# mic-rud/Learned-Compression-of-Point-Cloud-Geometry-and-Attributes

Hardware: AMD Instinct MI355X
Metric: encode+decode Mpoints/sec (higher is better)
Workload: dtype f32

## Files before the change

### include/pcc_hip.h

```cpp
#ifndef PCC_HIP_H
#define PCC_HIP_H

#include <stdint.h>

#ifdef __cplusplus
extern "C" {
#endif

#define PCC_OK 0
#define PCC_ERR_ARG (-1)
#define PCC_ERR_HIP (-2)
#define PCC_ERR_UNSUPPORTED (-3)
#define PCC_ERR_DATA (-4)

#define PCC_ACT_NONE 0
#define PCC_ACT_RELU 1
#define PCC_ACT_LEAKY_RELU 2

int pcc_version(void);
const char* pcc_last_error(void);
int pcc_device_count(void);
int pcc_device_name(int dev, char* out, int out_len);

int64_t pcc_hash_capacity(int64_t n);

#define PCC_COORD_LIMIT 130000
#define PCC_BATCH_LIMIT 1022
#define PCC_COUNT_ERR_RANGE (-2)

int pcc_hash_build(const int32_t* coords, int64_t n, uint64_t* keys, int32_t* vals, int64_t cap,
                   int32_t tensor_stride, int32_t* dup_count, void* stream);

int pcc_hash_lookup(const uint64_t* keys, const int32_t* vals, int64_t cap, int32_t tensor_stride,
                    const int32_t* query, int64_t nq, int32_t* out_idx, void* stream);

int64_t pcc_scan_scratch_elems(int64_t m);

int pcc_stride_map(const int32_t* coords, int64_t n, int32_t ts, uint64_t* keys, int32_t* vals,
                   int64_t cap, int32_t* scratch, int32_t* out_coords, int64_t* out_count,
                   void* stream);

int pcc_children(const int32_t* coords, int64_t n, int32_t ts, int32_t ksize, uint64_t* keys,
                 int32_t* vals, int64_t cap, int32_t* scratch, int32_t* out_coords,
                 int64_t* out_count, void* stream);

int pcc_kernel_map(const int32_t* out_coords, int64_t n_out, const uint64_t* in_keys,
                   const int32_t* in_vals, int64_t in_cap, int32_t ksize, int32_t step,
                   int32_t sign, int32_t* nbr, uint32_t* row_mask, int64_t* pair_count,
                   void* stream);

int pcc_pair_count(const uint32_t* row_mask, int64_t n_out, int64_t* pair_count, void* stream);

int64_t pcc_order_scratch_bytes(int64_t n);
int pcc_order_rows_by_mask(const uint32_t* row_mask, const int32_t* coords, int64_t n,
                           int32_t block_log2, int32_t tensor_stride, int32_t* order, uint32_t* group_mask32,
                           void* scratch, int64_t scratch_bytes, void* stream);
int pcc_permute_map_rows(const int32_t* nbr, const int32_t* order, int64_t n, int32_t K, int32_t* nbr_sorted, void* stream);

int64_t pcc_small_map_max(void);
int32_t pcc_small_paths(int32_t mask);
int pcc_small_kernel_map(const int32_t* out_coords, int64_t n_out, const uint64_t* in_keys, const int32_t* in_vals, int64_t in_cap,
                         int32_t ksize, int32_t step, int32_t sign, int32_t* nbr, uint32_t* row_mask, int32_t* order,
                         uint32_t* group_mask32, void* scratch, int64_t scratch_bytes, void* stream);

int64_t pcc_conv_packed_elems(int32_t K, int32_t cin, int32_t cout);
int pcc_conv_pack_weights(const float* w, int32_t K, int32_t cin, int32_t cout, float* w_packed,
                          void* stream);
int pcc_conv_fwd(const float* fin, int64_t n_in, int32_t cin, const float* w, const float* w_packed,
                 const float* bias, const int32_t* nbr, const int32_t* order,
                 const uint32_t* group_mask32, int32_t K, float* fout, int64_t n_out, int32_t cout,
                 int32_t act, const float* film, const float* residual, void* stream);

int64_t pcc_conv_small_max(int64_t workgroups);

int pcc_conv_kernel_name(int32_t mode, int64_t n_in, int32_t cin, int32_t cout, int64_t n_out, int32_t K, int32_t has_nbr,
                         char* buf, int32_t len);

int64_t pcc_conv_packed_elems_bf16(int32_t K, int32_t cin, int32_t cout);
int pcc_conv_pack_weights_bf16(const float* w, int32_t K, int32_t cin, int32_t cout, uint16_t* w_packed, void* stream);
int pcc_conv_fwd_bf16(const uint16_t* fin, int64_t n_in, int32_t cin, const uint16_t* w_packed, const float* bias,
                      const int32_t* nbr, const int32_t* order, const uint32_t* group_mask32, int32_t K, float* fout,
                      int64_t n_out, int32_t cout, int32_t act, const float* film, const float* residual, void* stream);

int pcc_epilogue_fwd(const float* c, const float* film, const float* residual, int64_t n, int32_t channels, int32_t act,
                     float* out, void* stream);
int pcc_epilogue_bwd(const float* dout, const float* c, const float* film, int64_t n, int32_t channels, int32_t act,
                     float* dc, float* dfilm, void* stream);

int64_t pcc_cast_colsum_scratch_elems(int32_t channels);
int pcc_cast_colsum(const float* x, int64_t n, int32_t channels, uint16_t* out_bf16, float* colsum, float* scratch,
// ... 96 lines not shown
```

### learned-compression-of-point-cloud-geometry-and-attributes_amd/_lib.py

```python
import ctypes
import os
import subprocess

_HERE = os.path.dirname(os.path.abspath(__file__))
SO_PATH = os.path.join(_HERE, "libpcc_hip.so")
_lib = None

c_void_p, c_int, c_i32, c_i64 = ctypes.c_void_p, ctypes.c_int, ctypes.c_int32, ctypes.c_int64

SIGNATURES = {
    "pcc_version": (c_int, []),
    "pcc_last_error": (ctypes.c_char_p, []),
    "pcc_device_count": (c_int, []),
    "pcc_device_name": (c_int, [c_int, ctypes.c_char_p, c_int]),
    "pcc_hash_capacity": (c_i64, [c_i64]),
    "pcc_hash_build": (c_int, [c_void_p, c_i64, c_void_p, c_void_p, c_i64, c_i32, c_void_p, c_void_p]),
    "pcc_hash_lookup": (c_int, [c_void_p, c_void_p, c_i64, c_i32, c_void_p, c_i64, c_void_p, c_void_p]),
    "pcc_scan_scratch_elems": (c_i64, [c_i64]),
    "pcc_stride_map": (c_int, [c_void_p, c_i64, c_i32, c_void_p, c_void_p, c_i64, c_void_p, c_void_p, c_void_p, c_void_p]),
    "pcc_children": (c_int, [c_void_p, c_i64, c_i32, c_i32, c_void_p, c_void_p, c_i64, c_void_p, c_void_p, c_void_p, c_void_p]),
    "pcc_kernel_map": (c_int, [c_void_p, c_i64, c_void_p, c_void_p, c_i64, c_i32, c_i32, c_i32, c_void_p, c_void_p, c_void_p, c_void_p]),
    "pcc_pair_count": (c_int, [c_void_p, c_i64, c_void_p, c_void_p]),
    "pcc_conv_packed_elems": (c_i64, [c_i32, c_i32, c_i32]),
    "pcc_conv_pack_weights": (c_int, [c_void_p, c_i32, c_i32, c_i32, c_void_p, c_void_p]),
    "pcc_order_scratch_bytes": (c_i64, [c_i64]),
    "pcc_order_rows_by_mask": (c_int, [c_void_p, c_void_p, c_i64, c_i32, c_i32, c_void_p, c_void_p, c_void_p, c_i64, c_void_p]),
    "pcc_permute_map_rows": (c_int, [c_void_p, c_void_p, c_i64, c_i32, c_void_p, c_void_p]),
    "pcc_conv_fwd": (c_int, [c_void_p, c_i64, c_i32, c_void_p, c_void_p, c_void_p, c_void_p, c_void_p, c_void_p, c_i32,
                             c_void_p, c_i64, c_i32, c_i32, c_void_p, c_void_p, c_void_p]),
    "pcc_conv_small_max": (c_i64, [c_i64]),
    "pcc_conv_kernel_name": (c_int, [c_i32, c_i64, c_i32, c_i32, c_i64, c_i32, c_i32, ctypes.c_char_p, c_i32]),
    "pcc_small_map_max": (c_i64, []),
    "pcc_small_paths": (c_i32, [c_i32]),
    "pcc_small_kernel_map": (c_int, [c_void_p, c_i64, c_void_p, c_void_p, c_i64, c_i32, c_i32, c_i32, c_void_p, c_void_p, c_void_p,
                                     c_void_p, c_void_p, c_i64, c_void_p]),
    "pcc_conv_packed_elems_bf16": (c_i64, [c_i32, c_i32, c_i32]),
    "pcc_conv_pack_weights_bf16": (c_int, [c_void_p, c_i32, c_i32, c_i32, c_void_p, c_void_p]),
    "pcc_conv_fwd_bf16": (c_int, [c_void_p, c_i64, c_i32, c_void_p, c_void_p, c_void_p, c_void_p, c_void_p, c_i32, c_void_p, c_i64,
                                  c_i32, c_i32, c_void_p, c_void_p, c_void_p]),
    "pcc_conv_packed_elems_x3": (c_i64, [c_i32, c_i32, c_i32]),
    "pcc_conv_pack_weights_x3": (c_int, [c_void_p, c_i32, c_i32, c_i32, c_void_p, c_void_p]),
    "pcc_conv_fwd_x3": (c_int, [c_void_p, c_i64, c_i32, c_void_p, c_void_p, c_void_p, c_void_p, c_void_p, c_i32, c_void_p, c_i64,
                                c_i32, c_i32, c_void_p, c_void_p, c_void_p]),
    "pcc_epilogue_fwd": (c_int, [c_void_p, c_void_p, c_void_p, c_i64, c_i32, c_i32, c_void_p, c_void_p]),
    "pcc_cast_colsum_scratch_elems": (c_i64, [c_i32]),
    "pcc_cast_colsum": (c_int, [c_void_p, c_i64, c_i32, c_void_p, c_void_p, c_void_p, c_i64, c_void_p]),
    "pcc_epilogue_bwd": (c_int, [c_void_p, c_void_p, c_void_p, c_i64, c_i32, c_i32, c_void_p, c_void_p, c_void_p]),
    "pcc_im2col_thin": (c_int, [c_void_p, c_i32, c_void_p, c_i64, c_i32, c_void_p, c_i32, c_void_p]),
    "pcc_gather_sum_fwd": (c_int, [c_void_p, c_i32, c_void_p, c_i32, c_i32, c_void_p, c_void_p, c_i64, c_i32, c_void_p]),
    "pcc_gather_rows": (c_int, [c_void_p, c_i32, c_void_p, c_i64, c_void_p, c_i32, c_void_p]),
    "pcc_scatter_rows": (c_int, [c_void_p, c_i32, c_void_p, c_i64, c_void_p, c_void_p]),
    "pcc_scatter_add_rows": (c_int, [c_void_p, c_i32, c_void_p, c_i64, c_void_p, c_void_p]),
    "pcc_compact_rows": (c_int, [c_void_p, c_i64, c_void_p, c_void_p, c_void_p, c_i32, c_void_p, c_void_p, c_void_p, c_void_p, c_void_p]),
    "pcc_topk_state_elems": (c_i64, [c_i32]),
    "pcc_topk_mask": (c_int, [c_void_p, c_i32, c_void_p, c_i64, c_i32, c_void_p, c_void_p, c_void_p, c_void_p]),
    "pcc_count_per_batch": (c_int, [c_void_p, c_i64, c_i32, c_void_p, c_void_p]),
    "pcc_sort_scratch_bytes": (c_i64, [c_i64]),
    "pcc_sort_coords": (c_int, [c_void_p, c_i64, c_void_p, c_void_p, c_i64, c_void_p]),
    "pcc_kernel_map_transpose": (c_int, [c_void_p, c_i64, c_i32, c_i64, c_void_p, c_void_p, c_void_p]),
    "pcc_conv_wgrad_scratch_elems": (c_i64, [c_i32, c_i32, c_i32]),
# ... 183 lines not shown
```

### learned-compression-of-point-cloud-geometry-and-attributes_amd/csrc/select.hip

```cpp
#include <stdlib.h>

#include "common.h"
#include "sort_small.h"

namespace pcc {

constexpr int TK_STRIDE = 264;
constexpr int TK_LDS_BATCHES = 16;

__device__ __forceinline__ uint32_t float_key(float v) {
    if (v != v) return 0xFFFFFFFFu;
    if (v == 0.0f) v = 0.0f;
    const uint32_t u = __float_as_uint(v);
    return (u & 0x80000000u) ? ~u : (u | 0x80000000u);
}

struct Key96 { uint32_t w[3]; };

__device__ __forceinline__ Key96 make_key(float logit, int4 c) {
    const uint64_t lo = ~pack_key(c.x, c.y, c.z, c.w);
    Key96 k;
    k.w[0] = float_key(logit);
    k.w[1] = (uint32_t)(lo >> 32);
    k.w[2] = (uint32_t)lo;
// ... 274 lines not shown
}

__global__ __launch_bounds__(256) void coords_to_keys(const int32_t* __restrict__ coords, int64_t n,
                                                      uint64_t* __restrict__ keys) {
    const int64_t i = (int64_t)blockIdx.x * 256 + threadIdx.x;
    if (i >= n) return;
    const int4 c = reinterpret_cast<const int4*>(coords)[i];
    keys[i] = pack_key(c.x, c.y, c.z, c.w);
}

__global__ __launch_bounds__(256) void mask_bit_counts_kernel(const uint32_t* __restrict__ row_mask, int64_t n,
                                                              uint32_t* __restrict__ counts) {
    __shared__ unsigned c[27];
    if (threadIdx.x < 27) c[threadIdx.x] = 0u;
    __syncthreads();
    unsigned mine[27];
#pragma unroll
    for (int b = 0; b < 27; ++b) mine[b] = 0u;
    for (int64_t i0 = (int64_t)blockIdx.x * 256; i0 < n; i0 += (int64_t)gridDim.x * 256) {
        const int64_t i = i0 + threadIdx.x;
        const uint32_t m = (i < n) ? row_mask[i] : 0u;
#pragma unroll
        for (int b = 0; b < 27; ++b) mine[b] += (unsigned)__popcll(__ballot((m >> b) & 1u));
    }
    if ((threadIdx.x & 63) == 0) {
#pragma unroll
        for (int b = 0; b < 27; ++b)
            if (mine[b]) atomicAdd(&c[b], mine[b]);
    }
    __syncthreads();
    if (threadIdx.x < 27 && c[threadIdx.x]) atomicAdd(&counts[threadIdx.x], c[threadIdx.x]);
}

__device__ __forceinline__ void order_bit_positions(const uint32_t* __restrict__ counts, int* pos_s) {
    if (threadIdx.x < 27) {
        const uint32_t mine = counts[threadIdx.x];
        int rank = 0;
        for (int b = 0; b < 27; ++b) {
            const uint32_t o = counts[b];
            rank += (o < mine || (o == mine && b < (int)threadIdx.x)) ? 1 : 0;
        }
        pos_s[threadIdx.x] = 26 - rank;
    }
    __syncthreads();
}

__device__ __forceinline__ uint32_t order_key_of(uint32_t m, const int* pos_s) {
    uint32_t key = 0u;
#pragma unroll
    for (int b = 0; b < 27; ++b) key |= ((m >> b) & 1u) << pos_s[b];
    return 0x7FFFFFFu - key;
}

__global__ __launch_bounds__(256) void order_keys32_kernel(const uint32_t* __restrict__ row_mask, int64_t n,
                                                           const uint32_t* __restrict__ counts, uint32_t* __restrict__ keys) {
    __shared__ int pos_s[27];
    order_bit_positions(counts, pos_s);
    const int64_t i = (int64_t)blockIdx.x * 256 + threadIdx.x;
    if (i >= n) return;
    const uint32_t m = row_mask[i] & 0x7FFFFFFu;
    keys[i] = order_key_of(m, pos_s);
}

__global__ __launch_bounds__(256) void order_keys64_kernel(const uint32_t* __restrict__ row_mask,
                                                           const int32_t* __restrict__ coords, int64_t n,
                                                           int block_log2, int ts, const uint32_t* __restrict__ counts,
                                                           uint64_t* __restrict__ keys) {
    __shared__ int pos_s[27];
    order_bit_positions(counts, pos_s);
    const int64_t i = (int64_t)blockIdx.x * 256 + threadIdx.x;
    if (i >= n) return;
    uint64_t key = order_key_of(row_mask[i] & 0x7FFFFFFu, pos_s);
    const int4 c = reinterpret_cast<const int4*>(coords)[i];
    const uint64_t bx = (uint64_t)(((c.y / ts) + 512) >> block_log2) & 0x3FF;
    const uint64_t by = (uint64_t)(((c.z / ts) + 512) >> block_log2) & 0x3FF;
    const uint64_t bz = (uint64_t)(((c.w / ts) + 512) >> block_log2) & 0x3FF;
    key |= ((((uint64_t)(c.x & 0x3) << 30) | (bx << 20) | (by << 10) | bz) << 32);
    keys[i] = key;
}

__global__ __launch_bounds__(256) void group_masks_kernel(const int32_t* __restrict__ order, const uint32_t* __restrict__ row_mask,
                                                          int64_t n, uint32_t* __restrict__ group_mask32) {
    const int64_t i = (int64_t)blockIdx.x * 256 + threadIdx.x;
    uint32_t m = (i < n) ? row_mask[order[i]] : 0u;
#pragma unroll
    for (int d = 1; d < 32; d <<= 1) m |= __shfl_xor(m, d, 64);
    if (i < n && (threadIdx.x & 31) == 0) group_mask32[i >> 5] = m;
}

__global__ __launch_bounds__(256) void permute_rows_kernel(const int32_t* __restrict__ order, const int32_t* __restrict__ nbr,
                                                           int64_t n, int K, int32_t* __restrict__ nbr_sorted) {
    __shared__ int32_t src_row[256];
    const int64_t r0 = (int64_t)blockIdx.x * 256;
    const int64_t i = r0 + threadIdx.x;
    src_row[threadIdx.x] = (i < n) ? order[i] : 0;
    __syncthreads();
    const int rows = (int)((n - r0 < 256) ? (n - r0) : 256);
    const int total = rows * K;
    int32_t* dst = nbr_sorted + r0 * K;
    for (int e = threadIdx.x; e < total; e += 256) {
        const int lr = e / K;
        const int k = e - lr * K;
        dst[e] = nbr[(int64_t)src_row[lr] * K + k];
    }
}


template <int ROUNDS>
__global__ __launch_bounds__(RS_SMALL_THREADS) void order_small_kernel(const uint32_t* __restrict__ row_mask, int n, uint32_t* keys_a,
                                                                      uint32_t* keys_b, int32_t* va, int32_t* vb) {
    __shared__ unsigned cnt27[27];
    __shared__ int pos_s[27];
    const int t = threadIdx.x;
    if (t < 27) cnt27[t] = 0u;
    __syncthreads();
    unsigned mine[27];
#pragma unroll
    for (int b = 0; b < 27; ++b) mine[b] = 0u;
    for (int i = t; i < n; i += RS_SMALL_THREADS) {
        const uint32_t m = row_mask[i];
// ... 159 lines not shown
        hipLaunchKernelGGL(topk_small_kernel, dim3(1), dim3(1024), 0, st, logits, ld, coords, (int)n, k, mask, state);
        PCC_LAUNCH_CHECK();
        return PCC_OK;
    }
    hipLaunchKernelGGL(topk_init, dim3(nbatch), dim3(256), 0, st, k, nbatch, state);
    if (n > 0) {
        const unsigned nb = blocks_for(n, 256, 512);
        if (nbatch == 1 && small_path_enabled(1)) {
            const unsigned groups = blocks_for(n, TK1_THREADS * 4, TK1_GROUPS);
            int32_t* partial = state + TK_STRIDE;
            for (int pass = 0; pass < 4; ++pass) {
                hipLaunchKernelGGL(topk_hist1_kernel, dim3(groups), dim3(TK1_THREADS), 0, st, logits, ld, n, pass, state, partial);
                hipLaunchKernelGGL(topk_pick1_kernel, dim3(1), dim3(1024), 0, st, pass, state, partial, (int)groups);
            }
            hipLaunchKernelGGL(topk_tail_kernel, dim3(1), dim3(1024), 0, st, logits, ld, coords, n, state);
            hipLaunchKernelGGL(topk_write_mask, dim3(blocks_for(n, 256)), dim3(256), 0, st, logits, ld, coords, n, nbatch,
                               state, mask);
            PCC_LAUNCH_CHECK();
            return PCC_OK;
        }
        for (int pass = 0; pass < 12; ++pass) {
            hipLaunchKernelGGL(topk_hist, dim3(nb), dim3(256), 0, st, logits, ld, coords, n, nbatch, pass, state);
            hipLaunchKernelGGL(topk_pick, dim3(nbatch), dim3(256), 0, st, pass, state);
        }
        hipLaunchKernelGGL(topk_write_mask, dim3(blocks_for(n, 256)), dim3(256), 0, st, logits, ld, coords, n, nbatch,
                           state, mask);
    }
    PCC_LAUNCH_CHECK();
    return PCC_OK;
}

int64_t pcc_order_scratch_bytes(int64_t n) { return pcc_sort_scratch_bytes(n); }

int pcc_order_rows_by_mask(const uint32_t* row_mask, const int32_t* coords, int64_t n, int32_t block_log2,
                           int32_t tensor_stride, int32_t* order, uint32_t* group_mask32, void* scratch, int64_t scratch_bytes,
                           void* stream) {
    if (n <= 0) return PCC_OK;
    PCC_REQUIRE(n < (1ll << 31), "pcc_order_rows_by_mask: too many rows");
    PCC_REQUIRE(block_log2 < 0 || coords != nullptr, "pcc_order_rows_by_mask: block ordering needs coordinates");
    PCC_REQUIRE(block_log2 <= 10, "pcc_order_rows_by_mask: block_log2 out of range");
    PCC_REQUIRE(tensor_stride >= 1, "pcc_order_rows_by_mask: bad tensor stride");
    PCC_REQUIRE(scratch_bytes >= pcc_sort_scratch_bytes(n), "pcc_order_rows_by_mask: scratch too small");
    hipStream_t st = as_stream(stream);
    char* p = reinterpret_cast<char*>(scratch);
    char* keys_a = p; p += align256(n * 8);
    char* keys_b = p; p += align256(n * 8);
    int32_t* vals_x = reinterpret_cast<int32_t*>(p); p += align256(n * 4);
    void* counters = p;
    uint32_t* bit_counts = reinterpret_cast<uint32_t*>(p + radix_sort_counter_bytes(n));
    if (small_path_enabled(0) && block_log2 < 0 && n <= RS_SMALL_N) {
        const int rounds = (int)(((n + RS_SMALL_WAVES - 1) / RS_SMALL_WAVES + 63) / 64);
        uint32_t* ka = reinterpret_cast<uint32_t*>(keys_a);
        uint32_t* kb = reinterpret_cast<uint32_t*>(keys_b);
#define PCC_ORDER_SMALL(R) hipLaunchKernelGGL(order_small_kernel<R>, dim3(1), dim3(RS_SMALL_THREADS), 0, st, row_mask, (int)n, ka, kb, vals_x, order)
        if (rounds <= 1) PCC_ORDER_SMALL(1);
        else if (rounds <= 2) PCC_ORDER_SMALL(2);
        else if (rounds <= 4) PCC_ORDER_SMALL(4);
        else if (rounds <= 8) PCC_ORDER_SMALL(8);
        else PCC_ORDER_SMALL(16);
#undef PCC_ORDER_SMALL
        hipLaunchKernelGGL(group_masks_kernel, dim3(blocks_for(n, 256)), dim3(256), 0, st, order, row_mask, n, group_mask32);
        PCC_LAUNCH_CHECK();
        return PCC_OK;
    }
    PCC_CHECK_HIP(hipMemsetAsync(bit_counts, 0, 27 * sizeof(uint32_t), st));
    hipLaunchKernelGGL(mask_bit_counts_kernel, dim3(blocks_for(n, 256 * 16, 512)), dim3(256), 0, st, row_mask, n, bit_counts);
    const int begin = 0, end = block_log2 >= 0 ? 64 : 27;
    const int digit_bits = block_log2 >= 0 ? 8 : radix_sort_order_digit_bits(n);
    const bool in_b = radix_sort_result_in_b(begin, end, digit_bits);
    int32_t* va = in_b ? vals_x : order;
    int32_t* vb = in_b ? order : vals_x;
    int rc;
    if (block_log2 < 0) {
        hipLaunchKernelGGL(order_keys32_kernel, dim3(blocks_for(n, 256)), dim3(256), 0, st, row_mask, n, bit_counts,
                           reinterpret_cast<uint32_t*>(keys_a));
        rc = radix_sort_pairs_u32(reinterpret_cast<uint32_t*>(keys_a), reinterpret_cast<uint32_t*>(keys_b), va, vb, true, n, begin, end,
                                  counters, st, digit_bits);
    } else {
        hipLaunchKernelGGL(order_keys64_kernel, dim3(blocks_for(n, 256)), dim3(256), 0, st, row_mask, coords, n, block_log2, tensor_stride,
                           bit_counts, reinterpret_cast<uint64_t*>(keys_a));
        rc = radix_sort_pairs_u64(reinterpret_cast<uint64_t*>(keys_a), reinterpret_cast<uint64_t*>(keys_b), va, vb, true, n, begin, end,
                                  counters, st);
    }
    if (rc) return rc;
    hipLaunchKernelGGL(group_masks_kernel, dim3(blocks_for(n, 256)), dim3(256), 0, st, order, row_mask, n, group_mask32);
    PCC_LAUNCH_CHECK();
    return PCC_OK;
}

int pcc_permute_map_rows(const int32_t* nbr, const int32_t* order, int64_t n, int32_t K, int32_t* nbr_sorted, void* stream) {
    PCC_REQUIRE(K >= 1 && K <= 27, "pcc_permute_map_rows: K out of range");
    PCC_REQUIRE(nbr != nullptr && order != nullptr && nbr_sorted != nullptr, "pcc_permute_map_rows: null argument");
    if (n <= 0) return PCC_OK;
    hipLaunchKernelGGL(permute_rows_kernel, dim3(blocks_for(n, 256)), dim3(256), 0, as_stream(stream), order, nbr, n, K, nbr_sorted);
    PCC_LAUNCH_CHECK();
    return PCC_OK;
}

int64_t pcc_sort_scratch_bytes(int64_t n) {
    if (n < 1) n = 1;
    return 2 * align256(n * 8) + align256(n * 4) + radix_sort_counter_bytes(n) + 256;
}

int pcc_sort_coords(const int32_t* coords, int64_t n, int32_t* perm, void* scratch, int64_t scratch_bytes, void* stream) {
    if (n <= 0) return PCC_OK;
    PCC_REQUIRE(n < (1ll << 31), "pcc_sort_coords: too many rows");
    PCC_REQUIRE(scratch_bytes >= pcc_sort_scratch_bytes(n), "pcc_sort_coords: scratch too small");
    hipStream_t st = as_stream(stream);
    char* p = reinterpret_cast<char*>(scratch);
    uint64_t* keys_a = reinterpret_cast<uint64_t*>(p); p += align256(n * 8);
    uint64_t* keys_b = reinterpret_cast<uint64_t*>(p); p += align256(n * 8);
    int32_t* vals_x = reinterpret_cast<int32_t*>(p); p += align256(n * 4);
    void* counters = p;
    hipLaunchKernelGGL(coords_to_keys, dim3(blocks_for(n, 256)), dim3(256), 0, st, coords, n, keys_a);
    const bool in_b = radix_sort_result_in_b(0, 64);
    return radix_sort_pairs_u64(keys_a, keys_b, in_b ? vals_x : perm, in_b ? perm : vals_x, true, n, 0, 64, counters, st);
}

// ... 2 lines not shown
```

### learned-compression-of-point-cloud-geometry-and-attributes_amd/csrc/sort.h

```cpp
#pragma once
#include "common.h"

namespace pcc {

static inline int64_t align256(int64_t v) { return (v + 255) / 256 * 256; }

int64_t scan_block_sums_elems(int64_t m);
int scan_flags(const int32_t* flags, int64_t m, int32_t* pos, int32_t* block_sums, int64_t* total, int inclusive,
               hipStream_t st, const int32_t* err = nullptr);

int radix_sort_passes(int begin_bit, int end_bit, int digit_bits = 8);
static inline bool radix_sort_result_in_b(int begin_bit, int end_bit, int digit_bits = 8) { return radix_sort_passes(begin_bit, end_bit, digit_bits) & 1; }
int64_t radix_sort_counter_bytes(int64_t n);
int radix_sort_order_digit_bits(int64_t n);
int radix_sort_pairs_u32(uint32_t* keys_a, uint32_t* keys_b, int32_t* vals_a, int32_t* vals_b, bool vals_are_iota, int64_t n,
                         int begin_bit, int end_bit, void* counters, hipStream_t st, int digit_bits = 8);
int radix_sort_pairs_u64(uint64_t* keys_a, uint64_t* keys_b, int32_t* vals_a, int32_t* vals_b, bool vals_are_iota, int64_t n,
                         int begin_bit, int end_bit, void* counters, hipStream_t st);

}
```

### learned-compression-of-point-cloud-geometry-and-attributes_amd/csrc/sort.hip

```cpp
#include "sort_small.h"

namespace pcc {

constexpr int RS_MID_ITEMS = 8;
constexpr int RS_MID_MAX_UNITS = 64;
constexpr int RS_BIG_ITEMS = 16;

template <class K, int ROUNDS, int DB>
__global__ __launch_bounds__(RS_SMALL_THREADS) void radix_sort_small_kernel(K* ka, K* kb, int32_t* va, int32_t* vb, int iota, int n,
                                                                           int begin_bit, int end_bit, int passes) {
    radix_sort_small_body<K, ROUNDS, DB>(ka, kb, va, vb, iota, n, begin_bit, end_bit, passes);
}

template <class K, int ITEMS, int DB>
__global__ __launch_bounds__(256) void radix_count_kernel(const K* __restrict__ keys, int64_t n, int shift, unsigned dmask,
                                                          int64_t nunits, int32_t* __restrict__ counts) {
    constexpr int ND = 1 << DB;
    __shared__ int cnt[ND];
#pragma unroll
    for (int d = threadIdx.x; d < ND; d += 256) cnt[d] = 0;
    __syncthreads();
    const int64_t base = (int64_t)blockIdx.x * (256 * ITEMS);
    K key[ITEMS];
#pragma unroll
    for (int j = 0; j < ITEMS; ++j) {
        const int64_t i = base + (int64_t)j * 256 + threadIdx.x;
        key[j] = (i < n) ? keys[i] : (K)0;
    }
#pragma unroll
    for (int j = 0; j < ITEMS; ++j)
        if (base + (int64_t)j * 256 + threadIdx.x < n) atomicAdd(&cnt[(unsigned)(key[j] >> shift) & dmask], 1);
    __syncthreads();
#pragma unroll
    for (int d = threadIdx.x; d < ND; d += 256) counts[(int64_t)d * nunits + blockIdx.x] = cnt[d];
}

__global__ __launch_bounds__(256) void radix_rowscan_kernel(int32_t* __restrict__ counts, int64_t nunits, int32_t* __restrict__ totals) {
    __shared__ int wsum[4];
    __shared__ int carry_s;
    const int t = threadIdx.x, lane = t & 63, w = t >> 6;
    int32_t* row = counts + (int64_t)blockIdx.x * nunits;
    if (t == 0) carry_s = 0;
    __syncthreads();
    for (int64_t base = 0; base < nunits; base += 1024) {
        const int64_t i = base + 4 * (int64_t)t;
        int f[4];
        int v = 0;
#pragma unroll
        for (int j = 0; j < 4; ++j) {
            f[j] = (i + j < nunits) ? row[i + j] : 0;
            v += f[j];
        }
        const int inc = wave_inclusive_scan_i32(v, lane);
        if (lane == 63) wsum[w] = inc;
        __syncthreads();
        int pre = carry_s;
        for (int ww = 0; ww < w; ++ww) pre += wsum[ww];
        int ex = pre + inc - v;
#pragma unroll
        for (int j = 0; j < 4; ++j) {
            if (i + j < nunits) row[i + j] = ex;
            ex += f[j];
        }
        __syncthreads();
        if (t == 255) carry_s = pre + inc;
        __syncthreads();
    }
    if (t == 0) totals[blockIdx.x] = carry_s;
}

template <class K, int ITEMS, bool SELF_PREFIX, int DB>
__global__ __launch_bounds__(256) void radix_scatter_kernel(const K* __restrict__ src, K* __restrict__ dst, const int32_t* __restrict__ vs,
                                                            int32_t* __restrict__ vd, int iota, int64_t n, int shift, unsigned dmask,
                                                            int64_t nunits, const int32_t* __restrict__ counts,
                                                            const int32_t* __restrict__ totals) {
    constexpr int WAVE_KEYS = 64 * ITEMS, WG_KEYS = 4 * WAVE_KEYS;
    constexpr int ND = 1 << DB, DH = ND / 256;
    __shared__ K skey[WG_KEYS];
    __shared__ int32_t sval[WG_KEYS];
    __shared__ int cnt[4][ND];
    __shared__ int lbase[ND];
    __shared__ int gbase[ND];
    __shared__ int wsum[4], wsum2[4];
    const int t = threadIdx.x, lane = t & 63, w = t >> 6;
    const uint64_t lt = (1ull << lane) - 1ull;
    for (int i = t; i < 4 * ND; i += 256) (&cnt[0][0])[i] = 0;
    const int64_t base0 = (int64_t)blockIdx.x * WG_KEYS;
    const int64_t wbase = base0 + (int64_t)w * WAVE_KEYS;
    K key[ITEMS];
    int32_t val[ITEMS];
#pragma unroll
    for (int j = 0; j < ITEMS; ++j) {
        const int64_t i = wbase + j * 64 + lane;
        key[j] = (i < n) ? src[i] : (K)0;
        val[j] = (i < n) ? (iota ? (int32_t)i : vs[i]) : 0;
    }
    int pre[DH], total[DH];
#pragma unroll
    for (int h = 0; h < DH; ++h) {
        const int d = h * 256 + t;
        if (SELF_PREFIX) {
            const int32_t* row = counts + (int64_t)d * nunits;
            pre[h] = 0;
            total[h] = 0;
            for (int64_t u = 0; u < nunits; ++u) {
                const int c = row[u];
                total[h] += c;
                pre[h] += (u < (int64_t)blockIdx.x) ? c : 0;
            }
        } else {
            pre[h] = counts[(int64_t)d * nunits + blockIdx.x];
            total[h] = totals[d];
        }
    }
    __syncthreads();
#pragma unroll
    for (int j = 0; j < ITEMS; ++j)
        if (wbase + j * 64 + lane < n) atomicAdd(&cnt[w][(unsigned)(key[j] >> shift) & dmask], 1);
    __syncthreads();
    int gcarry = 0, lcarry = 0;
#pragma unroll
    for (int h = 0; h < DH; ++h) {
        const int d = h * 256 + t;
        const int c0 = cnt[0][d], c1 = cnt[1][d], c2 = cnt[2][d], c3 = cnt[3][d];
        const int mine = c0 + c1 + c2 + c3;
        const int inc = wave_inclusive_scan_i32(total[h], lane);
        const int linc = wave_inclusive_scan_i32(mine, lane);
// ... 25 lines not shown
        }
        __builtin_amdgcn_wave_barrier();
        if (active && below == 0) cnt[w][d] = base + __popcll(same);
        __builtin_amdgcn_wave_barrier();
    }
    __syncthreads();
    const int nk = (int)((n - base0 < WG_KEYS) ? (n - base0) : WG_KEYS);
    for (int i = t; i < nk; i += 256) {
        const K k = skey[i];
        const unsigned d = (unsigned)(k >> shift) & dmask;
        const int64_t pos = (int64_t)gbase[d] + (i - lbase[d]);
        dst[pos] = k;
        vd[pos] = sval[i];
    }
}

int radix_sort_passes(int begin_bit, int end_bit, int digit_bits) {
    return end_bit > begin_bit ? (end_bit - begin_bit + digit_bits - 1) / digit_bits : 0;
}

int radix_sort_order_digit_bits(int64_t n) {
    const int64_t mid_units = (n + 256 * RS_MID_ITEMS - 1) / (256 * RS_MID_ITEMS);
    return (n > RS_SMALL_N && mid_units <= RS_MID_MAX_UNITS) ? 8 : 9;
}

int64_t radix_sort_counter_bytes(int64_t n) {
    const int64_t mid = (n + 256 * RS_MID_ITEMS - 1) / (256 * RS_MID_ITEMS), big = (n + 256 * RS_BIG_ITEMS - 1) / (256 * RS_BIG_ITEMS);
    const int64_t nunits = mid <= RS_MID_MAX_UNITS ? mid : big;
    return align256(512 * (nunits > 0 ? nunits : 1) * 4) + 2048;
}

template <class K, int DB>
static int radix_sort_pairs(K* ka, K* kb, int32_t* va, int32_t* vb, bool iota, int64_t n, int begin_bit, int end_bit, void* counters,
                            hipStream_t st) {
    constexpr int ND = 1 << DB;
    const int passes = radix_sort_passes(begin_bit, end_bit, DB);
    PCC_REQUIRE(passes >= 1 && end_bit <= (int)(8 * sizeof(K)) && begin_bit >= 0, "radix sort: bad bit range [%d, %d)", begin_bit, end_bit);
    PCC_REQUIRE(n < (1ll << 31), "radix sort: too many keys (%lld)", (long long)n);
    if (n <= 0) return PCC_OK;
    if (n <= RS_SMALL_N) {
        const int rounds = (int)(((n + RS_SMALL_WAVES - 1) / RS_SMALL_WAVES + 63) / 64);
#define PCC_RS_SMALL(R)                                                                                                             \
    hipLaunchKernelGGL((radix_sort_small_kernel<K, R, DB>), dim3(1), dim3(RS_SMALL_THREADS), 0, st, ka, kb, va, vb, iota ? 1 : 0, (int)n, \
                       begin_bit, end_bit, passes)
        if (rounds <= 1) PCC_RS_SMALL(1);
        else if (rounds <= 2) PCC_RS_SMALL(2);
        else if (rounds <= 4) PCC_RS_SMALL(4);
        else if (rounds <= 8) PCC_RS_SMALL(8);
        else PCC_RS_SMALL(16);
#undef PCC_RS_SMALL
        PCC_LAUNCH_CHECK();
        return PCC_OK;
    }
    const int64_t mid_units = (n + 256 * RS_MID_ITEMS - 1) / (256 * RS_MID_ITEMS);
    const bool mid = mid_units <= RS_MID_MAX_UNITS;
    const int64_t nunits = mid ? mid_units : (n + 256 * RS_BIG_ITEMS - 1) / (256 * RS_BIG_ITEMS);
    int32_t* counts = reinterpret_cast<int32_t*>(counters);
    int32_t* totals = counts + align256((int64_t)ND * nunits * 4) / 4;
    K* src = ka;
    K* dst = kb;
    int32_t* vs = va;
    int32_t* vd = vb;
    for (int p = 0; p < passes; ++p) {
        const int shift = begin_bit + DB * p;
        const unsigned dmask = (end_bit - shift >= DB) ? (unsigned)(ND - 1) : ((1u << (end_bit - shift)) - 1u);
        const int io = (iota && p == 0) ? 1 : 0;
        if (mid) {
            hipLaunchKernelGGL((radix_count_kernel<K, RS_MID_ITEMS, DB>), dim3((unsigned)nunits), dim3(256), 0, st, src, n, shift, dmask, nunits, counts);
            hipLaunchKernelGGL((radix_scatter_kernel<K, RS_MID_ITEMS, true, DB>), dim3((unsigned)nunits), dim3(256), 0, st, src, dst, vs, vd, io, n,
                               shift, dmask, nunits, counts, totals);
        } else {
            hipLaunchKernelGGL((radix_count_kernel<K, RS_BIG_ITEMS, DB>), dim3((unsigned)nunits), dim3(256), 0, st, src, n, shift, dmask, nunits, counts);
            hipLaunchKernelGGL(radix_rowscan_kernel, dim3(ND), dim3(256), 0, st, counts, nunits, totals);
            hipLaunchKernelGGL((radix_scatter_kernel<K, RS_BIG_ITEMS, false, DB>), dim3((unsigned)nunits), dim3(256), 0, st, src, dst, vs, vd, io, n,
                               shift, dmask, nunits, counts, totals);
        }
        K* tk = src; src = dst; dst = tk;
        int32_t* tv = vs; vs = vd; vd = tv;
    }
    PCC_LAUNCH_CHECK();
    return PCC_OK;
}

int radix_sort_pairs_u32(uint32_t* keys_a, uint32_t* keys_b, int32_t* vals_a, int32_t* vals_b, bool vals_are_iota, int64_t n, int begin_bit,
                         int end_bit, void* counters, hipStream_t st, int digit_bits) {
    if (digit_bits == 9) return radix_sort_pairs<uint32_t, 9>(keys_a, keys_b, vals_a, vals_b, vals_are_iota, n, begin_bit, end_bit, counters, st);
    return radix_sort_pairs<uint32_t, 8>(keys_a, keys_b, vals_a, vals_b, vals_are_iota, n, begin_bit, end_bit, counters, st);
}

int radix_sort_pairs_u64(uint64_t* keys_a, uint64_t* keys_b, int32_t* vals_a, int32_t* vals_b, bool vals_are_iota, int64_t n, int begin_bit,
                         int end_bit, void* counters, hipStream_t st) {
    return radix_sort_pairs<uint64_t, 8>(keys_a, keys_b, vals_a, vals_b, vals_are_iota, n, begin_bit, end_bit, counters, st);
}

}
```

### learned-compression-of-point-cloud-geometry-and-attributes_amd/sparse.py

```python
import ctypes
import functools
import math
import weakref

import os

import torch
import torch.nn as nn

from . import _lib, _threads
from ._lib import check, ptr

ACT_NONE, ACT_RELU, ACT_LRELU = 0, 1, 2


def _require_cuda(t):
    if not t.is_cuda:
        raise RuntimeError("libpcc_hip operators need tensors on an MI355X device (got a CPU tensor); "
                           "there is no CPU fallback")


COORD_PROFILER = None


# ... 18 lines not shown
    if coords.dtype.is_floating_point:
        coords = torch.floor(coords)
    return coords.to(torch.int32).contiguous()


def _host_count():
    st = _threads.current()
    if st.count is None:
        buf = torch.zeros(1, dtype=torch.int64, pin_memory=True)
        st.count = (buf, buf.numpy())
    st.count[1][0] = COUNT_ARMED
    return st.count


_SMALL_MAP_MAX = None


def _small_map_max():
    global _SMALL_MAP_MAX
    if _SMALL_MAP_MAX is None:
        _SMALL_MAP_MAX = int(_lib.lib().pcc_small_map_max())
    return _SMALL_MAP_MAX


def set_small_map_max(rows):
    global _SMALL_MAP_MAX
    was = _small_map_max()
    _SMALL_MAP_MAX = min(int(rows), int(_lib.lib().pcc_small_map_max())) if rows else 0
    return was


def set_small_paths(mask):
    return int(_lib.lib().pcc_small_paths(int(mask)))


class CoordinateRangeError(ValueError):
    """a coordinate outside the voxel key's range (|c| <= 130000, 0 <= batch index <= 1022: include/pcc_hip.h)"""


COUNT_ARMED, COUNT_ERR_RANGE = -1, -2


def _read_count(word, device):
    import time
    deadline = time.perf_counter() + 2e-3
    while word[0] == COUNT_ARMED:
        if time.perf_counter() > deadline:
            torch.cuda.current_stream(device).synchronize()
            break
        time.sleep(0)
    n = int(word[0])
    if n == COUNT_ERR_RANGE:
        raise CoordinateRangeError("libpcc_hip: a voxel coordinate is outside the supported range (|c| <= 130000, batch index "
                                   "<= 1022): the 18-bit fields of the voxel key would alias — translate the cloud towards the "
                                   "origin or re-voxelise it")
    if n < 0:
        raise RuntimeError("libpcc_hip: the row count was never written (kernel failure?)")
    return n


class PairCount:

    def __init__(self, row_mask):
        self._mask, self._val = row_mask, None

    def item(self):
# ... 738 lines not shown
```

Measured before the change: 8.775.

## Fuse order-key generation into first radix pass and derive group masks from sorted keys

For large row counts, the 27-bit order keys are now computed inside the first radix count and scatter passes straight from the row masks. This drops the separate key-building kernel and its write and read of the key array. Group masks are also rebuilt from the sorted keys using stored bit positions, instead of a gather through the order permutation back into the row masks, which avoids random reads. Both paths are on by default and can be turned off with environment variables. The cost is recomputing keys in both the count and scatter kernels, plus a small extra global buffer for bit positions.

```diff
diff --git a/include/pcc_hip.h b/include/pcc_hip.h
--- a/include/pcc_hip.h
+++ b/include/pcc_hip.h
@@ -56,6 +56,8 @@
                            int32_t block_log2, int32_t tensor_stride, int32_t* order, uint32_t* group_mask32,
                            void* scratch, int64_t scratch_bytes, void* stream);
 int pcc_permute_map_rows(const int32_t* nbr, const int32_t* order, int64_t n, int32_t K, int32_t* nbr_sorted, void* stream);
+
+int32_t pcc_order_paths(int32_t mask);
 
 int64_t pcc_small_map_max(void);
 int32_t pcc_small_paths(int32_t mask);
diff --git a/learned-compression-of-point-cloud-geometry-and-attributes_amd/_lib.py b/learned-compression-of-point-cloud-geometry-and-attributes_amd/_lib.py
--- a/learned-compression-of-point-cloud-geometry-and-attributes_amd/_lib.py
+++ b/learned-compression-of-point-cloud-geometry-and-attributes_amd/_lib.py
@@ -26,6 +26,7 @@
     "pcc_order_scratch_bytes": (c_i64, [c_i64]),
     "pcc_order_rows_by_mask": (c_int, [c_void_p, c_void_p, c_i64, c_i32, c_i32, c_void_p, c_void_p, c_void_p, c_i64, c_void_p]),
     "pcc_permute_map_rows": (c_int, [c_void_p, c_void_p, c_i64, c_i32, c_void_p, c_void_p]),
+    "pcc_order_paths": (c_i32, [c_i32]),
     "pcc_conv_fwd": (c_int, [c_void_p, c_i64, c_i32, c_void_p, c_void_p, c_void_p, c_void_p, c_void_p, c_void_p, c_i32,
                              c_void_p, c_i64, c_i32, c_i32, c_void_p, c_void_p, c_void_p]),
     "pcc_conv_small_max": (c_i64, [c_i64]),
diff --git a/learned-compression-of-point-cloud-geometry-and-attributes_amd/csrc/select.hip b/learned-compression-of-point-cloud-geometry-and-attributes_amd/csrc/select.hip
--- a/learned-compression-of-point-cloud-geometry-and-attributes_amd/csrc/select.hip
+++ b/learned-compression-of-point-cloud-geometry-and-attributes_amd/csrc/select.hip
@@ -330,30 +330,12 @@
     if (threadIdx.x < 27 && c[threadIdx.x]) atomicAdd(&counts[threadIdx.x], c[threadIdx.x]);
 }
 
-__device__ __forceinline__ void order_bit_positions(const uint32_t* __restrict__ counts, int* pos_s) {
-    if (threadIdx.x < 27) {
-        const uint32_t mine = counts[threadIdx.x];
-        int rank = 0;
-        for (int b = 0; b < 27; ++b) {
-            const uint32_t o = counts[b];
-            rank += (o < mine || (o == mine && b < (int)threadIdx.x)) ? 1 : 0;
-        }
-        pos_s[threadIdx.x] = 26 - rank;
-    }
-    __syncthreads();
-}
-
-__device__ __forceinline__ uint32_t order_key_of(uint32_t m, const int* pos_s) {
-    uint32_t key = 0u;
-#pragma unroll
-    for (int b = 0; b < 27; ++b) key |= ((m >> b) & 1u) << pos_s[b];
-    return 0x7FFFFFFu - key;
-}
-
 __global__ __launch_bounds__(256) void order_keys32_kernel(const uint32_t* __restrict__ row_mask, int64_t n,
-                                                           const uint32_t* __restrict__ counts, uint32_t* __restrict__ keys) {
+                                                           const uint32_t* __restrict__ counts, int32_t* __restrict__ bit_pos,
+                                                           uint32_t* __restrict__ keys) {
     __shared__ int pos_s[27];
     order_bit_positions(counts, pos_s);
+    if (blockIdx.x == 0 && threadIdx.x < 27) bit_pos[threadIdx.x] = pos_s[threadIdx.x];
     const int64_t i = (int64_t)blockIdx.x * 256 + threadIdx.x;
     if (i >= n) return;
     const uint32_t m = row_mask[i] & 0x7FFFFFFu;
@@ -363,9 +345,10 @@
 __global__ __launch_bounds__(256) void order_keys64_kernel(const uint32_t* __restrict__ row_mask,
                                                            const int32_t* __restrict__ coords, int64_t n,
                                                            int block_log2, int ts, const uint32_t* __restrict__ counts,
-                                                           uint64_t* __restrict__ keys) {
+                                                           int32_t* __restrict__ bit_pos, uint64_t* __restrict__ keys) {
     __shared__ int pos_s[27];
     order_bit_positions(counts, pos_s);
+    if (blockIdx.x == 0 && threadIdx.x < 27) bit_pos[threadIdx.x] = pos_s[threadIdx.x];
     const int64_t i = (int64_t)blockIdx.x * 256 + threadIdx.x;
     if (i >= n) return;
     uint64_t key = order_key_of(row_mask[i] & 0x7FFFFFFu, pos_s);
@@ -384,6 +367,31 @@
 #pragma unroll
     for (int d = 1; d < 32; d <<= 1) m |= __shfl_xor(m, d, 64);
     if (i < n && (threadIdx.x & 31) == 0) group_mask32[i >> 5] = m;
+}
+
+template <class K>
+__global__ __launch_bounds__(256) void group_masks_sorted_kernel(const K* __restrict__ sorted_keys, const int32_t* __restrict__ bit_pos,
+                                                                 int64_t n, uint32_t* __restrict__ group_mask32) {
+    constexpr int ITEMS = 8;
+    __shared__ int pos_s[27];
+    const int64_t base = (int64_t)blockIdx.x * (256 * ITEMS);
+    uint32_t perm[ITEMS];
+#pragma unroll
+    for (int j = 0; j < ITEMS; ++j) {
+        const int64_t i = base + j * 256 + threadIdx.x;
+        perm[j] = (i < n) ? 0x7FFFFFFu - ((uint32_t)sorted_keys[i] & 0x7FFFFFFu) : 0u;
+    }
+    order_bit_positions_stored(bit_pos, pos_s);
+    const int b = threadIdx.x & 31;
+    const int mypos = b < 27 ? pos_s[b] : 31;
+#pragma unroll
+    for (int j = 0; j < ITEMS; ++j) {
+#pragma unroll
+        for (int d = 1; d < 32; d <<= 1) perm[j] |= __shfl_xor(perm[j], d, 64);
+        const uint64_t both = __ballot((perm[j] >> mypos) & 1u);
+        const int64_t i = base + j * 256 + threadIdx.x;
+        if (i < n && b == 0) group_mask32[i >> 5] = (uint32_t)((threadIdx.x & 32) ? (both >> 32) : both);
+    }
 }
 
 __global__ __launch_bounds__(256) void permute_rows_kernel(const int32_t* __restrict__ order, const int32_t* __restrict__ nbr,
@@ -609,6 +617,28 @@
 
 int64_t pcc_order_scratch_bytes(int64_t n) { return pcc_sort_scratch_bytes(n); }
 
+constexpr int64_t ORDER_SORTED_MASKS_MIN_ROWS = 2000000;
+
+static int g_order_paths = -1;
+static int order_paths_value() {
+    if (g_order_paths < 0) {
+        const char* names[2] = {"PCC_ORDER_SORTED_MASKS", "PCC_ORDER_FUSED_KEYS"};
+        int v = 0;
+        for (int b = 0; b < 2; ++b) {
+            const char* e = getenv(names[b]);
+            if (!(e && e[0] == '0')) v |= 1 << b;
+        }
+        g_order_paths = v;
+    }
+    return g_order_paths;
+}
+
+int32_t pcc_order_paths(int32_t mask) {
+    const int before = order_paths_value();
+    if (mask >= 0) g_order_paths = mask & 3;
+    return before;
+}
+
 int pcc_order_rows_by_mask(const uint32_t* row_mask, const int32_t* coords, int64_t n, int32_t block_log2,
                            int32_t tensor_stride, int32_t* order, uint32_t* group_mask32, void* scratch, int64_t scratch_bytes,
                            void* stream) {
@@ -642,6 +672,8 @@
     }
     PCC_CHECK_HIP(hipMemsetAsync(bit_counts, 0, 27 * sizeof(uint32_t), st));
     hipLaunchKernelGGL(mask_bit_counts_kernel, dim3(blocks_for(n, 256 * 16, 512)), dim3(256), 0, st, row_mask, n, bit_counts);
+    int32_t* bit_pos = reinterpret_cast<int32_t*>(bit_counts + 32);
+    const int paths = order_paths_value();
     const int begin = 0, end = block_log2 >= 0 ? 64 : 27;
     const int digit_bits = block_log2 >= 0 ? 8 : radix_sort_order_digit_bits(n);
     const bool in_b = radix_sort_result_in_b(begin, end, digit_bits);
@@ -649,18 +681,33 @@
     int32_t* vb = in_b ? order : vals_x;
     int rc;
     if (block_log2 < 0) {
-        hipLaunchKernelGGL(order_keys32_kernel, dim3(blocks_for(n, 256)), dim3(256), 0, st, row_mask, n, bit_counts,
-                           reinterpret_cast<uint32_t*>(keys_a));
-        rc = radix_sort_pairs_u32(reinterpret_cast<uint32_t*>(keys_a), reinterpret_cast<uint32_t*>(keys_b), va, vb, true, n, begin, end,
-                                  counters, st, digit_bits);
+        if ((paths & 2) && n > radix_sort_small_limit()) {
+            rc = radix_sort_order_from_masks(row_mask, bit_counts, bit_pos, reinterpret_cast<uint32_t*>(keys_a), reinterpret_cast<uint32_t*>(keys_b),
+                                             va, vb, n, counters, st, digit_bits);
+        } else {
+            hipLaunchKernelGGL(order_keys32_kernel, dim3(blocks_for(n, 256)), dim3(256), 0, st, row_mask, n, bit_counts, bit_pos,
+                               reinterpret_cast<uint32_t*>(keys_a));
+            rc = radix_sort_pairs_u32(reinterpret_cast<uint32_t*>(keys_a), reinterpret_cast<uint32_t*>(keys_b), va, vb, true, n, begin,
+                                      end, counters, st, digit_bits);
+        }
     } else {
         hipLaunchKernelGGL(order_keys64_kernel, dim3(blocks_for(n, 256)), dim3(256), 0, st, row_mask, coords, n, block_log2, tensor_stride,
-                           bit_counts, reinterpret_cast<uint64_t*>(keys_a));
+                           bit_counts, bit_pos, reinterpret_cast<uint64_t*>(keys_a));
         rc = radix_sort_pairs_u64(reinterpret_cast<uint64_t*>(keys_a), reinterpret_cast<uint64_t*>(keys_b), va, vb, true, n, begin, end,
                                   counters, st);
     }
     if (rc) return rc;
-    hipLaunchKernelGGL(group_masks_kernel, dim3(blocks_for(n, 256)), dim3(256), 0, st, order, row_mask, n, group_mask32);
+    if ((paths & 1) && n > ORDER_SORTED_MASKS_MIN_ROWS) {
+        const unsigned nb = blocks_for(n, 256 * 8);
+        if (block_log2 < 0)
+            hipLaunchKernelGGL(group_masks_sorted_kernel<uint32_t>, dim3(nb), dim3(256), 0, st,
+                               reinterpret_cast<const uint32_t*>(in_b ? keys_b : keys_a), bit_pos, n, group_mask32);
+        else
+            hipLaunchKernelGGL(group_masks_sorted_kernel<uint64_t>, dim3(nb), dim3(256), 0, st,
+                               reinterpret_cast<const uint64_t*>(in_b ? keys_b : keys_a), bit_pos, n, group_mask32);
+    } else {
+        hipLaunchKernelGGL(group_masks_kernel, dim3(blocks_for(n, 256)), dim3(256), 0, st, order, row_mask, n, group_mask32);
+    }
     PCC_LAUNCH_CHECK();
     return PCC_OK;
 }
diff --git a/learned-compression-of-point-cloud-geometry-and-attributes_amd/csrc/sort.h b/learned-compression-of-point-cloud-geometry-and-attributes_amd/csrc/sort.h
--- a/learned-compression-of-point-cloud-geometry-and-attributes_amd/csrc/sort.h
+++ b/learned-compression-of-point-cloud-geometry-and-attributes_amd/csrc/sort.h
@@ -18,4 +18,35 @@
 int radix_sort_pairs_u64(uint64_t* keys_a, uint64_t* keys_b, int32_t* vals_a, int32_t* vals_b, bool vals_are_iota, int64_t n,
                          int begin_bit, int end_bit, void* counters, hipStream_t st);
 
+#ifdef __HIPCC__
+__device__ __forceinline__ void order_bit_positions(const uint32_t* counts, int* pos_s) {
+    if (threadIdx.x < 27) {
+        const uint32_t mine = counts[threadIdx.x];
+        int rank = 0;
+        for (int b = 0; b < 27; ++b) {
+            const uint32_t o = counts[b];
+            rank += (o < mine || (o == mine && b < (int)threadIdx.x)) ? 1 : 0;
+        }
+        pos_s[threadIdx.x] = 26 - rank;
+    }
+    __syncthreads();
 }
+
+__device__ __forceinline__ void order_bit_positions_stored(const int32_t* __restrict__ pos_g, int* pos_s) {
+    if (threadIdx.x < 27) pos_s[threadIdx.x] = pos_g[threadIdx.x];
+    __syncthreads();
+}
+
+__device__ __forceinline__ uint32_t order_key_of(uint32_t m, const int* pos_s) {
+    uint32_t key = 0u;
+#pragma unroll
+    for (int b = 0; b < 27; ++b) key |= ((m >> b) & 1u) << pos_s[b];
+    return 0x7FFFFFFu - key;
+}
+#endif
+
+int64_t radix_sort_small_limit();
+int radix_sort_order_from_masks(const uint32_t* row_mask, const uint32_t* counts, int32_t* bit_pos, uint32_t* keys_a, uint32_t* keys_b,
+                                int32_t* vals_a, int32_t* vals_b, int64_t n, void* counters, hipStream_t st, int digit_bits);
+
+}
diff --git a/learned-compression-of-point-cloud-geometry-and-attributes_amd/csrc/sort.hip b/learned-compression-of-point-cloud-geometry-and-attributes_amd/csrc/sort.hip
--- a/learned-compression-of-point-cloud-geometry-and-attributes_amd/csrc/sort.hip
+++ b/learned-compression-of-point-cloud-geometry-and-attributes_amd/csrc/sort.hip
@@ -12,11 +12,18 @@
     radix_sort_small_body<K, ROUNDS, DB>(ka, kb, va, vb, iota, n, begin_bit, end_bit, passes);
 }
 
-template <class K, int ITEMS, int DB>
+template <class K, int ITEMS, int DB, bool MASKS = false>
 __global__ __launch_bounds__(256) void radix_count_kernel(const K* __restrict__ keys, int64_t n, int shift, unsigned dmask,
-                                                          int64_t nunits, int32_t* __restrict__ counts) {
+                                                          int64_t nunits, int32_t* __restrict__ counts,
+                                                          const uint32_t* __restrict__ bit_counts = nullptr,
+                                                          int32_t* __restrict__ bit_pos = nullptr) {
     constexpr int ND = 1 << DB;
     __shared__ int cnt[ND];
+    __shared__ int pos_s[MASKS ? 27 : 1];
+    if (MASKS) {
+        order_bit_positions(bit_counts, pos_s);
+        if (blockIdx.x == 0 && threadIdx.x < 27) bit_pos[threadIdx.x] = pos_s[threadIdx.x];
+    }
 #pragma unroll
     for (int d = threadIdx.x; d < ND; d += 256) cnt[d] = 0;
     __syncthreads();
@@ -26,6 +33,7 @@
     for (int j = 0; j < ITEMS; ++j) {
         const int64_t i = base + (int64_t)j * 256 + threadIdx.x;
         key[j] = (i < n) ? keys[i] : (K)0;
+        if (MASKS) key[j] = (K)order_key_of((uint32_t)key[j] & 0x7FFFFFFu, pos_s);
     }
 #pragma unroll
     for (int j = 0; j < ITEMS; ++j)
@@ -69,11 +77,12 @@
     if (t == 0) totals[blockIdx.x] = carry_s;
 }
 
-template <class K, int ITEMS, bool SELF_PREFIX, int DB>
+template <class K, int ITEMS, bool SELF_PREFIX, int DB, bool MASKS = false>
 __global__ __launch_bounds__(256) void radix_scatter_kernel(const K* __restrict__ src, K* __restrict__ dst, const int32_t* __restrict__ vs,
                                                             int32_t* __restrict__ vd, int iota, int64_t n, int shift, unsigned dmask,
                                                             int64_t nunits, const int32_t* __restrict__ counts,
-                                                            const int32_t* __restrict__ totals) {
+                                                            const int32_t* __restrict__ totals,
+                                                            const int32_t* __restrict__ bit_pos = nullptr) {
     constexpr int WAVE_KEYS = 64 * ITEMS, WG_KEYS = 4 * WAVE_KEYS;
     constexpr int ND = 1 << DB, DH = ND / 256;
     __shared__ K skey[WG_KEYS];
@@ -82,8 +91,10 @@
     __shared__ int lbase[ND];
     __shared__ int gbase[ND];
     __shared__ int wsum[4], wsum2[4];
+    __shared__ int pos_s[MASKS ? 27 : 1];
     const int t = threadIdx.x, lane = t & 63, w = t >> 6;
     const uint64_t lt = (1ull << lane) - 1ull;
+    if (MASKS) order_bit_positions_stored(bit_pos, pos_s);
     for (int i = t; i < 4 * ND; i += 256) (&cnt[0][0])[i] = 0;
     const int64_t base0 = (int64_t)blockIdx.x * WG_KEYS;
     const int64_t wbase = base0 + (int64_t)w * WAVE_KEYS;
@@ -93,6 +104,7 @@
     for (int j = 0; j < ITEMS; ++j) {
         const int64_t i = wbase + j * 64 + lane;
         key[j] = (i < n) ? src[i] : (K)0;
+        if (MASKS) key[j] = (K)order_key_of((uint32_t)key[j] & 0x7FFFFFFu, pos_s);
         val[j] = (i < n) ? (iota ? (int32_t)i : vs[i]) : 0;
     }
     int pre[DH], total[DH];
@@ -184,12 +196,13 @@
 
 template <class K, int DB>
 static int radix_sort_pairs(K* ka, K* kb, int32_t* va, int32_t* vb, bool iota, int64_t n, int begin_bit, int end_bit, void* counters,
-                            hipStream_t st) {
+                            hipStream_t st, const uint32_t* masks = nullptr, const uint32_t* bit_counts = nullptr, int32_t* bit_pos = nullptr) {
     constexpr int ND = 1 << DB;
     const int passes = radix_sort_passes(begin_bit, end_bit, DB);
     PCC_REQUIRE(passes >= 1 && end_bit <= (int)(8 * sizeof(K)) && begin_bit >= 0, "radix sort: bad bit range [%d, %d)", begin_bit, end_bit);
     PCC_REQUIRE(n < (1ll << 31), "radix sort: too many keys (%lld)", (long long)n);
     if (n <= 0) return PCC_OK;
+    PCC_REQUIRE(masks == nullptr || (sizeof(K) == 4 && n > RS_SMALL_N), "radix sort: keys from masks need the multi-workgroup shapes");
     if (n <= RS_SMALL_N) {
         const int rounds = (int)(((n + RS_SMALL_WAVES - 1) / RS_SMALL_WAVES + 63) / 64);
 #define PCC_RS_SMALL(R)                                                                                                             \
@@ -217,7 +230,23 @@
         const int shift = begin_bit + DB * p;
         const unsigned dmask = (end_bit - shift >= DB) ? (unsigned)(ND - 1) : ((1u << (end_bit - shift)) - 1u);
         const int io = (iota && p == 0) ? 1 : 0;
-        if (mid) {
+        if (masks && p == 0) {
+            if constexpr (sizeof(K) == 4) {
+                const K* mk = reinterpret_cast<const K*>(masks);
+                if (mid) {
+                    hipLaunchKernelGGL((radix_count_kernel<K, RS_MID_ITEMS, DB, true>), dim3((unsigned)nunits), dim3(256), 0, st, mk, n, shift, dmask,
+                                       nunits, counts, bit_counts, bit_pos);
+                    hipLaunchKernelGGL((radix_scatter_kernel<K, RS_MID_ITEMS, true, DB, true>), dim3((unsigned)nunits), dim3(256), 0, st, mk, dst, vs,
+                                       vd, io, n, shift, dmask, nunits, counts, totals, bit_pos);
+                } else {
+                    hipLaunchKernelGGL((radix_count_kernel<K, RS_BIG_ITEMS, DB, true>), dim3((unsigned)nunits), dim3(256), 0, st, mk, n, shift, dmask,
+                                       nunits, counts, bit_counts, bit_pos);
+                    hipLaunchKernelGGL(radix_rowscan_kernel, dim3(ND), dim3(256), 0, st, counts, nunits, totals);
+                    hipLaunchKernelGGL((radix_scatter_kernel<K, RS_BIG_ITEMS, false, DB, true>), dim3((unsigned)nunits), dim3(256), 0, st, mk, dst,
+                                       vs, vd, io, n, shift, dmask, nunits, counts, totals, bit_pos);
+                }
+            }
+        } else if (mid) {
             hipLaunchKernelGGL((radix_count_kernel<K, RS_MID_ITEMS, DB>), dim3((unsigned)nunits), dim3(256), 0, st, src, n, shift, dmask, nunits, counts);
             hipLaunchKernelGGL((radix_scatter_kernel<K, RS_MID_ITEMS, true, DB>), dim3((unsigned)nunits), dim3(256), 0, st, src, dst, vs, vd, io, n,
                                shift, dmask, nunits, counts, totals);
@@ -240,6 +269,15 @@
     return radix_sort_pairs<uint32_t, 8>(keys_a, keys_b, vals_a, vals_b, vals_are_iota, n, begin_bit, end_bit, counters, st);
 }
 
+int64_t radix_sort_small_limit() { return RS_SMALL_N; }
+
+int radix_sort_order_from_masks(const uint32_t* row_mask, const uint32_t* counts, int32_t* bit_pos, uint32_t* keys_a, uint32_t* keys_b,
+                                int32_t* vals_a, int32_t* vals_b, int64_t n, void* counters, hipStream_t st, int digit_bits) {
+    if (digit_bits == 9)
+        return radix_sort_pairs<uint32_t, 9>(keys_a, keys_b, vals_a, vals_b, true, n, 0, 27, counters, st, row_mask, counts, bit_pos);
+    return radix_sort_pairs<uint32_t, 8>(keys_a, keys_b, vals_a, vals_b, true, n, 0, 27, counters, st, row_mask, counts, bit_pos);
+}
+
 int radix_sort_pairs_u64(uint64_t* keys_a, uint64_t* keys_b, int32_t* vals_a, int32_t* vals_b, bool vals_are_iota, int64_t n, int begin_bit,
                          int end_bit, void* counters, hipStream_t st) {
     return radix_sort_pairs<uint64_t, 8>(keys_a, keys_b, vals_a, vals_b, vals_are_iota, n, begin_bit, end_bit, counters, st);
diff --git a/learned-compression-of-point-cloud-geometry-and-attributes_amd/sparse.py b/learned-compression-of-point-cloud-geometry-and-attributes_amd/sparse.py
--- a/learned-compression-of-point-cloud-geometry-and-attributes_amd/sparse.py
+++ b/learned-compression-of-point-cloud-geometry-and-attributes_amd/sparse.py
@@ -74,6 +74,10 @@
 
 def set_small_paths(mask):
     return int(_lib.lib().pcc_small_paths(int(mask)))
+
+
+def set_order_paths(mask):
+    return int(_lib.lib().pcc_order_paths(int(mask)))
 
 
 class CoordinateRangeError(ValueError):
```

New measurement: 8.758 (median of 2 runs). About the same (-0.2%).
